# pairlab/SlotFormer

Hardware: AMD Instinct MI355X
Metric: rollout frames/sec at B=32, 128x128, 7 slots, 6+50 steps (SAVi-encode + SlotFormer rollout) (higher is better)
Workload: dtype f32 storage; matmul/conv on split-bf16 MFMA (bf16x3: hi*hi+hi*lo+lo*hi, f32 accumulate)

## Files before the change

include/slotformer_hip.h:

```cpp
#ifndef SLOTFORMER_HIP_H
#define SLOTFORMER_HIP_H
#include <stddef.h>

#ifdef __cplusplus
extern "C" {
#endif

int sf_version(void);
const char* sf_last_error_string(void);

int sf_get_precision(void);
int sf_set_precision(int mode);

int sf_profile_enable(int class_mask);
int sf_set_seam_fused(int on);
int sf_get_seam_fused(void);
int sf_set_ffn_rows64(int on);
int sf_get_ffn_rows64(void);
int sf_profile_sample(int every);
int sf_profile_read(int kernel_class, double* total_ms, long long* launches, double* work);


int sf_linear_f32(const float* A, int lda, const float* W, const float* bias, const float* ln_gamma,
                  const float* ln_beta, float ln_eps, const float* residual, int ldr, float* C, int ldc,
// ... 55 lines not shown
                        const float* std3, float* out, int F, int H0, int W0, int H, int W, int antialias, int max_blocks, void* stream);
int sf_resize_masks_nearest(const void* src, int src_is_u8, const void* tables, long long* out_i64, unsigned char* out_u8, int F, int H0,
                            int W0, int H, int W, void* stream);

enum { SF_EGRESS_TRUNC = 0, SF_EGRESS_NEAREST_EVEN = 1 };
enum { SF_EGRESS_F32_CHW = 0, SF_EGRESS_U8_CHW = 1, SF_EGRESS_U8_HWC = 2 };
enum { SF_EGRESS_IMG = 0, SF_EGRESS_SLOTS = 1, SF_EGRESS_IDS = 2 };
int sf_egress_frames_u8(const float* x, unsigned char* out, long long F, int H, int W, int hwc, int to_rgb, int rounding, void* stream);
typedef struct {
  int kind;
  int N;
  const void* a;
  const void* b;
  float scale;
  int ids_i64;
  int P;
  int history_len;
} sf_egress_tile;
int sf_egress_grid_shape(int K, int H, int W, int nrow, int padding, int border, int* CH, int* CW);
int sf_egress_grid(const sf_egress_tile* tiles, int n_entries, void* out, int out_mode, int T, int H, int W, int nrow, int padding,
                   float pad_value, int border, void* stream);
int sf_egress_draw_boxes(unsigned char* frames, const float* boxes, const unsigned char* pres, const unsigned char* palette, int P, int F, int M,
                         int H, int W, int width, void* stream);

int sf_pos_embed_table_f32(const float* grid, const float* dense_w, const float* dense_b, float* table, int HW,
                           int C, void* stream);

int sf_slot_attn_num_partials(int HW);
int sf_slot_attn_iter_f32(const float* k, const float* v, int ld, long long batch_stride, const float* q,
                          float* part_num, float* part_den, float* attn_out, int B, int HW, int N, int D,
                          float scale, float eps, void* stream);

int sf_slot_attn_iter_bf16(const void* k, const void* v, int ld, long long batch_stride, const float* q, float* part_num,
                           float* part_den, float* attn_out, int B, int HW, int N, int D, float scale, float eps, void* stream);

size_t sf_slot_attn_iter_bwd_workspace_bytes(int B, int HW, int N, int D);
int sf_slot_attn_iter_bwd_f32(const float* k, const float* v, int ld, long long batch_stride, const float* q,
                              const float* part_num, const float* part_den, int P, const float* d_updates, float* dk,
                              float* dv, int accumulate, float* dq, int B, int HW, int N, int D, float scale, float eps,
                              void* ws, size_t ws_bytes, void* stream);

int sf_slot_update_f32(const float* part_num, const float* part_den, int P, const float* slots_prev,
                       const float* gru_w_ih, const float* gru_w_hh, const float* gru_b_ih,
                       const float* gru_b_hh, const float* ln_g, const float* ln_b, const float* mlp_w1,
                       const float* mlp_b1, const float* mlp_w2, const float* mlp_b2, float* slots_out, int B,
                       int N, int D, int H, float ln_eps, void* stream);

int sf_slot_update_packed_f32(const float* part_num, const float* part_den, int P, const float* slots_prev,
                              const void* gru_ih_packed, const void* gru_hh_packed, const float* gru_b_ih,
                              const float* gru_b_hh, const float* ln_g, const float* ln_b, const void* mlp_w1_packed,
                              const float* mlp_b1, const void* mlp_w2_packed, const float* mlp_b2, float* slots_out,
                              const float* q_ln_g, const float* q_ln_b, const void* q_w_packed, float* q_out, int B, int N,
                              int D, int H, float ln_eps, void* stream);

int sf_mha_f32(const float* qkv, float* out, int B, int L, int Lq, int d_model, int num_heads, void* stream);

int sf_qkv_attention_f32(const float* x, const float* ln_gamma, const float* ln_beta, float ln_eps,
                         const float* in_proj_w, const float* in_proj_b, float* out, int B, int L, int Lq, int d_model,
                         int num_heads, void* stream);

int sf_lstm_pointwise_f32(const float* gates, const float* c_prev, float* h_out, float* c_out, int R, int H,
                          void* stream);

int sf_sample_dist_f32(const float* dist, const float* noise, float* out, int R, int D, void* stream);

int sf_bilinear_resize_f32(const float* in, float* out, long long R, int Hi, int Wi, int Ho, int Wo,
                           void* stream);

size_t sf_groupnorm1_workspace_bytes(int F);
int sf_groupnorm1_nhwc_f32(const float* x, const float* gamma, const float* beta, float* y, int F, int H, int W, int C,
                           float eps, int relu, int pixel_shuffle, void* ws, size_t ws_bytes, void* stream);
size_t sf_groupnorm1_bwd_workspace_bytes(int F, int H, int W, int C);
int sf_groupnorm1_nhwc_bwd_f32(const float* x, const float* gamma, const float* beta, const float* dy, float* dx, float* dgamma,
                               float* dbeta, int F, int H, int W, int C, float eps, int relu, int pixel_shuffle, void* ws,
                               size_t ws_bytes, void* stream);

int sf_slate_attention_f32(const float* q, const float* k, const float* v, float* out, int ldq, int ldk, int ldv, int ldo,
                           int B, int Lq, int Lk, int num_heads, int head_dim, int causal, void* stream);
size_t sf_slate_attention_bwd_workspace_bytes(int B, int Lq, int num_heads);
int sf_slate_attention_train_fwd_f32(const float* q, const float* k, const float* v, float* out, float* lse, int ldq, int ldk,
                                     int ldv, int ldo, long long q_bs, long long k_bs, long long v_bs, long long o_bs, int B,
                                     int Lq, int Lk, int num_heads, int head_dim, int causal, float dropout_p,
                                     unsigned long long seed, void* stream);
int sf_slate_attention_train_bwd_f32(const float* q, const float* k, const float* v, const float* out, const float* d_out,
                                     const float* lse, float* dq, float* dk, float* dv, int ldq, int ldk, int ldv, int ldo,
                                     long long q_bs, long long k_bs, long long v_bs, long long o_bs, int B, int Lq, int Lk,
                                     int num_heads, int head_dim, int causal, float dropout_p, unsigned long long seed, void* ws,
                                     size_t ws_bytes, void* stream);
int sf_slate_attention_bwd_f32(const float* q, const float* k, const float* v, const float* out, const float* d_out, float* dq,
                               float* dk, float* dv, int ldq, int ldk, int ldv, int ldo, long long q_bs, long long k_bs,
                               long long v_bs, long long o_bs, int B, int Lq, int Lk, int num_heads, int head_dim, int causal,
                               void* ws, size_t ws_bytes, void* stream);
int sf_slate_attention_strided_f32(const float* q, const float* k, const float* v, float* out, int ldq, int ldk, int ldv,
                                   int ldo, long long q_bs, long long k_bs, long long v_bs, long long o_bs, int B, int Lq,
                                   int Lk, int num_heads, int head_dim, int causal, void* stream);
int sf_embed_tokens_f32(const long long* idx, const float* tok_emb, const float* pos, float* out, int B, int L, int d,
                        void* stream);
int sf_argmax_rows_f32(const float* x, long long ld, long long* out, long long R, int V, void* stream);
int sf_cross_entropy_f32(const float* x, const long long* target, float* loss_rows, float* mean_out, long long R, int V,
                         void* stream);
int sf_softmax_rows_f32(const float* x, const float* add, float scale, float* y, long long R, int V, void* stream);
int sf_cross_entropy_bwd_f32(const float* x, const long long* target, const float* g, float* dx, long long R, int V, void* stream);
int sf_log_softmax_rows_f32(const float* x, float* y, long long R, int V, void* stream);
int sf_gumbel_softmax_rows_f32(const float* x, unsigned long long seed, float scale, float* y, long long R, int V, void* stream);
int sf_softmax_rows_bwd_f32(const float* y, const float* dy, float scale, float* dx, long long R, int V, void* stream);

// ... 322 lines not shown
```

slotformer_amd/_lib.py:

```python
import ctypes as C
import os

_HERE = os.path.dirname(os.path.abspath(__file__))
LIB_PATH = os.environ.get('SF_LIB_PATH') or os.path.join(_HERE, 'libslotformer_hip.so')

FP = C.c_void_p


class sf_tfm_layer(C.Structure):
    _fields_ = [(n, FP) for n in (
        'norm1_g', 'norm1_b', 'in_proj_w', 'in_proj_b', 'out_proj_w', 'out_proj_b',
        'norm2_g', 'norm2_b', 'lin1_w', 'lin1_b', 'lin2_w', 'lin2_b', 'lin1_packed', 'lin2_packed', 'attn_in_packed', 'attn_out_packed', 'tok_packed')]


class sf_rollouter(C.Structure):
    _fields_ = [(n, C.c_int) for n in (
        'num_slots', 'slot_size', 'd_model', 'num_layers', 'num_heads', 'ffn_dim', 'norm_first',
        'window_len', 'single_step')] + [(n, FP) for n in (
            'in_proj_w', 'in_proj_b', 'out_proj_w', 'out_proj_b', 'pe_tok')] + [
                ('layers', C.POINTER(sf_tfm_layer)), ('in_proj_packed', C.c_void_p), ('out_proj_packed', C.c_void_p)]


class sf_rollout_opts(C.Structure):
    _fields_ = [(n, C.c_int) for n in ('precision', 'seam_fused', 'ffn_rows', 'attn_heads_per_wg', 'attn_qkv_rows', 'ffn_tile', 'cus_available', 'layer_tok')]
# ... 100 lines not shown
    'sf_set_precision': (I, [I]),
    'sf_profile_enable': (I, [I]),
    'sf_profile_sample': (I, [I]),
    'sf_set_seam_fused': (I, [I]),
    'sf_get_seam_fused': (I, []),
    'sf_set_ffn_rows64': (I, [I]),
    'sf_get_ffn_rows64': (I, []),
    'sf_profile_read': (I, [I, C.POINTER(C.c_double), C.POINTER(C.c_longlong), C.POINTER(C.c_double)]),
    'sf_linear_f32': (I, [FP, I, FP, FP, FP, FP, F32, FP, I, FP, I, I, I, I, I, VP]),
    'sf_layernorm_f32': (I, [FP, FP, FP, FP, I, I, F32, VP]),
    'sf_conv2d_nchw_in_f32': (I, [FP, LL, FP, FP, FP, FP, I, I, I, I, I, I, I, I, VP]),
    'sf_conv2d_nhwc_f32': (I, [FP, FP, FP, FP, FP, I, I, I, I, I, I, I, VP]),
    'sf_pack_conv_weight_f32': (I, [FP, FP, I, I, I, VP]),
    'sf_pixel_feat_f32': (I, [FP] * 10 + [I, F32, I, VP]),
    'sf_conv_frag_bytes': (SZ, [I, I, I]),
    'sf_set_conv_fp16x2': (I, [I]),
    'sf_get_conv_fp16x2': (I, []),
    'sf_pack_conv_frag_weights': (I, [FP, VP, I, I, I, VP]),
    'sf_conv5x5_frag_f32': (I, [FP, VP, FP, FP, FP, I, I, I, I, VP]),
    'sf_conv5x5_ws_f32': (I, [FP, VP, FP, FP, FP, I, I, I, I, I, VP]),
    'sf_deconv_frag_bytes': (SZ, [I, I, I, I]),
    'sf_pack_deconv_frag_weights': (I, [FP, VP, I, I, I, I, VP]),
    'sf_deconv5x5s2_frag_f32': (I, [FP, VP, FP, FP, I, I, I, I, VP]),
    'sf_deconv5x5s2_head_frag_f32': (I, [FP, VP, FP, FP, FP, FP, I, I, I, VP]),
    'sf_decode_l0_expand_f32': (I, [FP, FP, FP, I, I, I, VP]),
    'sf_conv_transpose2d_nhwc_f32': (I, [FP, FP, FP, FP, I, I, I, I, I, I, I, I, VP]),
    'sf_pack_deconv_weight_f32': (I, [FP, FP, I, I, I, VP]),
    'sf_slot_broadcast_f32': (I, [FP, FP, FP, I, I, I, VP]),
    'sf_decode_combine_f32': (I, [FP, FP, FP, FP, I, I, I, VP]),
    'sf_savi_decode_workspace_bytes': (SZ, [C.POINTER(sf_savi_decoder), I]),
    'sf_savi_decode_f32': (I, [C.POINTER(sf_savi_decoder), FP, FP, FP, FP, I, VP, SZ, VP]),
    'sf_savi_decode_seg_f32': (I, [C.POINTER(sf_savi_decoder), FP, FP, FP, FP, VP, VP, F32, I, VP, SZ, VP]),
    'sf_decode_combine_seg_f32': (I, [FP, FP, FP, FP, VP, VP, F32, VP, I, I, I, VP]),
    'sf_postproc_mask_f32': (I, [FP, VP, VP, F32, VP, I, I, I, VP]),
    'sf_vp_metrics_workspace_bytes': (SZ, [I, I, I]),
    'sf_vp_image_metrics_f32': (I, [FP, FP, VP, VP, VP, I, I, I, I, VP, SZ, VP]),
    'sf_vp_mask_metrics': (I, [VP, VP, I, VP, FP, VP, VP, VP, VP, I, I, I, I, VP, SZ, VP]),
    'sf_vp_bbox_pr_f32': (I, [FP, VP, FP, VP, VP, I, I, I, F32, VP]),
    'sf_masks_to_boxes': (I, [VP, I, FP, VP, I, I, I, I, VP]),
    'sf_vp_mean_over_videos_f64': (I, [VP, VP, I, I, I, VP]),
    'sf_ingest_tables_bytes': (SZ, [I, I, I, I, I]),
    'sf_ingest_tables_host': (I, [VP, SZ, I, I, I, I, I]),
    'sf_ingest_frames_u8': (I, [VP, VP, I, VP, FP, FP, FP, I, I, I, I, I, I, I, VP]),
    'sf_resize_masks_nearest': (I, [VP, I, VP, VP, VP, I, I, I, I, I, VP]),
    'sf_egress_frames_u8': (I, [FP, VP, LL, I, I, I, I, I, VP]),
    'sf_egress_grid_shape': (I, [I, I, I, I, I, I, C.POINTER(I), C.POINTER(I)]),
    'sf_egress_grid': (I, [C.POINTER(sf_egress_tile), I, VP, I, I, I, I, I, I, F32, I, VP]),
    'sf_egress_draw_boxes': (I, [VP, FP, VP, VP, I, I, I, I, I, I, VP]),
    'sf_pos_embed_table_f32': (I, [FP, FP, FP, FP, I, I, VP]),
    'sf_slot_attn_num_partials': (I, [I]),
    'sf_slot_attn_iter_f32': (I, [FP, FP, I, LL, FP, FP, FP, FP, I, I, I, I, F32, F32, VP]),
    'sf_slot_update_f32': (I, [FP, FP, I, FP] + [FP] * 10 + [FP, I, I, I, I, F32, VP]),
    'sf_slot_update_packed_f32': (I, [FP, FP, I, FP, VP, VP, FP, FP, FP, FP, VP, FP, VP, FP, FP, FP, FP, VP, FP, I, I, I, I, F32, VP]),
    'sf_mha_f32': (I, [FP, FP, I, I, I, I, I, VP]),
    'sf_qkv_attention_f32': (I, [FP, FP, FP, F32, FP, FP, FP, I, I, I, I, I, VP]),
    'sf_lstm_pointwise_f32': (I, [FP, FP, FP, FP, I, I, VP]),
    'sf_sample_dist_f32': (I, [FP, FP, FP, I, I, VP]),
    'sf_bilinear_resize_f32': (I, [FP, FP, LL, I, I, I, I, VP]),
    'sf_rollout_workspace_bytes': (SZ, [C.POINTER(sf_rollouter), I]),
    'sf_rollout_f32': (I, [C.POINTER(sf_rollouter), FP, I, I, I, VP, SZ, VP]),
    'sf_rollout_opts_f32': (I, [C.POINTER(sf_rollouter), FP, I, I, I, VP, SZ, VP, C.POINTER(sf_rollout_opts)]),
    'sf_rollout_uses_seam': (I, [C.POINTER(sf_rollouter), I]),
    'sf_rollout_uses_seam_opts': (I, [C.POINTER(sf_rollouter), I, C.POINTER(sf_rollout_opts)]),
    'sf_rollout_is_fused': (I, [C.POINTER(sf_rollouter)]),
    'sf_rollout_tok_ok': (I, [C.POINTER(sf_rollouter)]),
    'sf_rollout_tok_layers': (I, [C.POINTER(sf_rollouter), I, C.POINTER(sf_rollout_opts)]),
    'sf_ffn_chunk_partials_f32': (I, [C.POINTER(sf_tfm_layer), FP, LL, FP, LL, I, I, I, VP]),
    'sf_attn_block_f32': (I, [C.POINTER(sf_tfm_layer), FP, FP, I, I, I, I, VP]),
    'sf_ffn_block_rows_f32': (I, [C.POINTER(sf_tfm_layer), FP, FP, I, I, VP]),
    'sf_set_layer_tok': (I, [I]),
    'sf_get_layer_tok': (I, []),
    'sf_layer_tok_packed_bytes': (SZ, []),
    'sf_layer_tok_packed_bytes_ex': (SZ, [I, I, I]),
    'sf_pack_layer_tok_weights': (I, [C.POINTER(sf_tfm_layer), VP, I, I, I, VP]),
    'sf_layer_tok_block_f32': (I, [C.POINTER(sf_tfm_layer), I, FP, FP, I, I, VP]),
    'sf_layer_tok_block_ex_f32': (I, [C.POINTER(sf_tfm_layer), I, I, I, I, FP, FP, I, I, VP]),
    'sf_debug_read_ts_layer_tok': (I, [C.POINTER(C.c_longlong)]),
    'sf_attn_rows_planes_bytes': (SZ, [I]),
    'sf_attn_block_rows_f32': (I, [C.POINTER(sf_tfm_layer), FP, FP, VP, I, I, I, VP]),
    'sf_slot_attn_iter_bwd_workspace_bytes': (SZ, [I, I, I, I]),
    'sf_slot_attn_iter_bwd_f32': (I, [FP, FP, I, LL, FP, FP, FP, I, FP, FP, FP, I, FP, I, I, I, I, F32, F32, VP, SZ, VP]),
    'sf_slot_attention_train_workspace_bytes': (SZ, [C.POINTER(sf_slot_attention), I, I, I]),
    'sf_slot_attention_train_fwd_f32': (I, [C.POINTER(sf_slot_attention), FP, FP, I, I, I, FP, VP, SZ, VP]),
    'sf_slot_attention_train_bwd_f32': (I, [C.POINTER(sf_slot_attention), FP, FP, FP, FP, C.POINTER(sf_slot_attention_grads), I, I, I,
                                            VP, SZ, VP]),
    'sf_savi_decode_train_workspace_bytes': (SZ, [C.POINTER(sf_savi_decoder), I]),
    'sf_savi_decode_train_fwd_f32': (I, [C.POINTER(sf_savi_decoder), FP, FP, FP, FP, I, VP, SZ, VP]),
    'sf_savi_decode_train_bwd_f32': (I, [C.POINTER(sf_savi_decoder), C.POINTER(C.c_void_p), FP, FP, FP, C.POINTER(sf_savi_decoder_grads),
                                         I, VP, SZ, VP]),
    'sf_savi_features_train_workspace_bytes': (SZ, [C.POINTER(sf_savi_features), I]),
    'sf_savi_features_train_fwd_f32': (I, [C.POINTER(sf_savi_features), FP, LL, I, FP, VP, SZ, VP]),
    'sf_savi_features_train_bwd_f32': (I, [C.POINTER(sf_savi_features), FP, LL, FP, C.POINTER(sf_savi_features_grads), I, VP, SZ, VP]),
    'sf_linear_bwd_workspace_bytes': (SZ, [LL, I, I]),
    'sf_linear_bwd_f32': (I, [FP, FP, FP, FP, FP, FP, FP, LL, I, I, I, VP, SZ, VP]),
    'sf_mha_train_fwd_f32': (I, [FP, FP, I, I, I, I, F32, C.c_ulonglong, VP]),
    'sf_mha_train_bwd_f32': (I, [FP, FP, FP, I, I, I, I, F32, C.c_ulonglong, VP]),
    'sf_dropout_f32': (I, [FP, FP, FP, LL, F32, C.c_ulonglong, VP]),
    'sf_adam_flat_f32': (I, [FP, FP, FP, FP, LL, I, F32, F32, F32, F32, VP]),
    'sf_grad_norm_workspace_bytes': (SZ, [LL]),
    'sf_grad_clip_coef_f32': (I, [FP, LL, F32, FP, VP, SZ, VP]),
    'sf_adam_flat_groups_f32': (I, [FP, FP, FP, FP, LL, I, C.POINTER(sf_adam_group), I, F32, F32, F32, FP, VP]),
    'sf_layernorm_bwd_workspace_bytes': (SZ, [I]),
    'sf_layernorm_bwd_f32': (I, [FP, FP, FP, FP, FP, FP, LL, I, F32, VP, SZ, VP]),
    'sf_rollout_train_workspace_bytes': (SZ, [C.POINTER(sf_rollouter), I, I]),
    'sf_rollout_train_fwd_f32': (I, [C.POINTER(sf_rollouter), FP, FP, I, I, F32, C.c_ulonglong, VP, SZ, VP]),
    'sf_rollout_train_bwd_f32': (I, [C.POINTER(sf_rollouter), FP, FP, C.POINTER(sf_rollouter_grads), I, I, F32,
# ... 177 lines not shown
```

slotformer_amd/csrc/slot_attn.hip:

```cpp
#include "sf_internal.h"
#include <stdlib.h>

#define SA_NMAX 8
#define SA_DMAX 256
#define SA_HMAX 512


template <int CTRL>
__device__ __forceinline__ float dpp_mov(float v) {
  return __int_as_float(__builtin_amdgcn_update_dpp(0, __float_as_int(v), CTRL, 0xf, 0xf, true));
}

__device__ __forceinline__ float wave_allsum(float v) {
  v += dpp_mov<0xB1>(v);
  v += dpp_mov<0x4E>(v);
  v += dpp_mov<0x141>(v);
  v += dpp_mov<0x140>(v);
  v += __shfl_xor(v, 16, 64);
  v += __shfl_xor(v, 32, 64);
  return v;
}

template <int VPT>
__global__ __launch_bounds__(256) void sa_attn_partial_kernel(
// ... 542 lines not shown
      const float v = su_sum(s_pa, ks, D2, j, r) + a.kd_b[j];
      s_hid[j * SU_R + r] = v;
      if (a.kdist_out && row < R) a.kdist_out[(long long)(row / N) * a.kdist_bs + (long long)(row % N) * D2 + j] = v;
    }
  }
  __syncthreads();
  for (int idx = t; idx < SU_R * D; idx += nt) {
    const int r = idx / D, d = idx - r * D, row = row0 + r;
    float v = s_hid[d * SU_R + r];
    if (a.noise && row < R)
      v += a.noise[(long long)(row / N) * a.noise_bs + (long long)(row % N) * D + d] * expf(s_hid[(D + d) * SU_R + r] * 0.5f);
    s_x[d * SU_R + r] = v;
    if (row < R) a.slots_out[(long long)row * D + d] = v;
  }
  __syncthreads();
  su_ln_stats(s_x, s_stat, D, ln_eps, wave, lane, nwaves);
  __syncthreads();
  for (int idx = t; idx < SU_R * D; idx += nt) {
    const int d = idx / SU_R, r = idx - d * SU_R;
    s_ln[idx] = (s_x[idx] - s_stat[2 * r]) * s_stat[2 * r + 1] * a.q_ln_g[d] + a.q_ln_b[d];
  }
  __syncthreads();
  su_gemm(a.q_w_t, D, D, s_ln, s_pa, t, nt);
  __syncthreads();
  {
    const int ks = su_kslices(nt, D, D);
    for (int idx = t; idx < SU_R * D; idx += nt) {
      const int r = idx / D, d = idx - r * D;
      if (row0 + r < R) a.q_out[(long long)(row0 + r) * D + d] = su_sum(s_pa, ks, D, d, r);
    }
  }
}

int sf_slot_prologue_ex(const float* prev, const float* init, const float* pm_ln_g, const float* pm_ln_b, const float* pm_w0_t,
                        const float* pm_b0, const float* pm_w2_t, const float* pm_b2, int norm_first, const float* kd_w_t,
                        const float* kd_b, const float* noise, long long noise_bs, float* kdist_out, long long kdist_bs,
                        const float* q_ln_g, const float* q_ln_b, const float* q_w_t, float* slots_out, float* q_out, int B,
                        int N, int D, float ln_eps, hipStream_t st) {
  if ((D % 64) != 0 || 2 * D > 768 || !kd_w_t || !kd_b || !q_w_t || !q_ln_g || !q_ln_b || !slots_out || !q_out || !init) return 1;
  if (prev && (!pm_ln_g || !pm_ln_b || !pm_w0_t || !pm_b0 || !pm_w2_t || !pm_b2)) return 1;
  if (B == 0) return 0;
  const int threads = 768, R = B * N, D2 = 2 * D;
  auto pmaxf = [&](int Nout, int K) { return su_kslices(threads, Nout, K) * Nout * SU_R; };
  int pmax = pmaxf(D2, D);
  if (pmaxf(D, D2) > pmax) pmax = pmaxf(D, D2);
  if (pmaxf(D, D) > pmax) pmax = pmaxf(D, D);
  const size_t lds = ((size_t)3 * D * SU_R + (size_t)D2 * SU_R + 2 * SU_R + (size_t)pmax) * sizeof(float);
  SF_TRY(sf_ensure_dyn_lds((const void*)sa_slot_prologue_kernel, lds));
  SpArgs a{prev, init, pm_ln_g, pm_ln_b, pm_w0_t, pm_b0, pm_w2_t, pm_b2, norm_first, kd_w_t, kd_b, noise, noise_bs, kdist_out,
           kdist_bs, q_ln_g, q_ln_b, q_w_t, slots_out, q_out};
  hipLaunchKernelGGL(sa_slot_prologue_kernel, dim3((R + SU_R - 1) / SU_R), dim3(threads), lds, st, a, R, N, D, pmax, ln_eps);
  SF_CHECK_LAUNCH();
  return 0;
}

int sf_sa_pick_partials(int HW) {
  if (HW % 256 == 0) return HW / 256;
  int P = HW / 128;
  while (P > 1 && (HW % P != 0 || (HW / P) % 16 != 0)) --P;
  if (P < 1) P = 1;
  return P;
}

extern "C" {

int sf_slot_attn_num_partials(int HW) { return sf_sa_pick_partials(HW); }

int sf_slot_attn_iter_f32(const float* k, const float* v, int ld, long long batch_stride, const float* q,
                          float* part_num, float* part_den, float* attn_out, int B, int HW, int N, int D,
                          float scale, float eps, void* stream) {
  return sf_slot_attn_iter_ex(k, v, ld, batch_stride, q, part_num, part_den, attn_out, (long long)N * HW, B, HW,
                              N, D, scale, eps, (hipStream_t)stream);
}
}

extern "C" int sf_slot_attn_iter_bf16(const void* k, const void* v, int ld, long long batch_stride, const float* q,
                                      float* part_num, float* part_den, float* attn_out, int B, int HW, int N, int D, float scale,
                                      float eps, void* stream) {
  SF_REQUIRE(k && v && q && part_num && part_den, "null pointer");
  SF_REQUIRE(B >= 0 && HW > 0 && (HW % 256) == 0 && N >= 1 && N <= SA_NMAX, "need 1 <= num_slots <= 8 and HW % 256 == 0");
  SF_REQUIRE(D == 64 || D == 128 || D == 192 || D == 256, "slot_size must be 64/128/192/256");
  SF_REQUIRE(ld >= D && (ld % 4) == 0 && (batch_stride % 4) == 0, "k/v rows must be 8-byte aligned");
  if (B == 0) return 0;
  const int P = sf_sa_pick_partials(HW);
  hipStream_t st = (hipStream_t)stream;
  dim3 grid(P, B), block(256);
  const __bf16* kb = (const __bf16*)k;
  const __bf16* vb = (const __bf16*)v;
  const long long abs_ = (long long)N * HW;
  sf_prof_begin(SF_K_SA_ITER, st, 2.0 * (double)B * HW * D * sizeof(__bf16));
#define SA_LAUNCHB(DD)                                                                                                   \
  hipLaunchKernelGGL((sa_attn_mfma_kernel<DD, __bf16>), grid, block, 0, st, kb, vb, ld, batch_stride, q, scale, eps, part_num, \
                     part_den, attn_out, abs_, HW, N, P)
  switch (D / 64) {
    case 1: SA_LAUNCHB(64); break;
    case 2: SA_LAUNCHB(128); break;
    case 3: SA_LAUNCHB(192); break;
    default: SA_LAUNCHB(256); break;
  }
#undef SA_LAUNCHB
  sf_prof_end(SF_K_SA_ITER, st);
  SF_CHECK_LAUNCH();
  return 0;
}

__device__ long long sa_ts[16];
// ... 225 lines not shown
```

slotformer_amd/csrc/slot_update_body.h:

```cpp
#pragma once
#include "sf_internal.h"


typedef float f32x16 __attribute__((ext_vector_type(16)));
typedef float f32x4 __attribute__((ext_vector_type(4)));
typedef __bf16 bf16x4 __attribute__((ext_vector_type(4)));
typedef __bf16 bf16x8 __attribute__((ext_vector_type(8)));

#ifdef UM_STAMPS
__device__ long long um_ts[16];
#define UMTS(i) do { if (block == 0 && threadIdx.x == 0) um_ts[i] = wall_clock64(); } while (0)
#else
#define UMTS(i) do { } while (0)
#endif

namespace {

constexpr int UM_D = 128, UM_H = 256, UM_ROWS = 32, UM_NT = 512;
constexpr int UM_DP = UM_D + 8, UM_HP = UM_H + 8;
constexpr int UM_FP = UM_D + 4;
constexpr int UV_BIH = 0, UV_BHH = 3 * UM_D, UV_LNG = 6 * UM_D, UV_LNB = 7 * UM_D, UV_B1 = 8 * UM_D, UV_B2 = 8 * UM_D + UM_H,
              UV_QG = 9 * UM_D + UM_H, UV_QB = 10 * UM_D + UM_H, UM_NV = 11 * UM_D + UM_H;
constexpr int UV_PG = UM_NV, UV_PBT = UV_PG + UM_D, UV_PB0 = UV_PBT + UM_D, UV_PB2 = UV_PB0 + UM_H, UV_KB = UV_PB2 + UM_D, UM_NV_NEXT = UV_KB + 2 * UM_D;
constexpr int UM_KP = 2 * UM_D + 8;
// ... 38 lines not shown
    acc = __builtin_amdgcn_mfma_f32_32x32x16_bf16(f.w[k][0], xl, acc, 0, 0, 0);
    acc = __builtin_amdgcn_mfma_f32_32x32x16_bf16(f.w[k][1], xh, acc, 0, 0, 0);
    acc = __builtin_amdgcn_mfma_f32_32x32x16_bf16(f.w[k][0], xh, acc, 0, 0, 0);
  }
}

struct UmArgs {
  const float *part_num, *part_den;
  int P;
  int pstep;
  const float* slots_prev;
  const uint4 *w_ih_p, *w_hh_p;
  const float *b_ih, *b_hh, *ln_g, *ln_b;
  const uint4* w1_p;
  const float* b1;
  const uint4* w2_p;
  const float* b2;
  float* slots_out;
  float* out2;
  long long out2_bs;
  const float *q_ln_g, *q_ln_b;
  const uint4* q_w_p;
  float* q_out;
  int R, N;
  float ln_eps;
  const float *pm_ln_g, *pm_ln_b;
  const uint4* pm_w0_p;
  const float* pm_b0;
  const uint4* pm_w2_p;
  const float* pm_b2;
  int pm_norm_first;
  const uint4* kd_w_p;
  const float* kd_b;
  const float* noise;
  long long noise_bs;
  float* kdist_out;
  long long kdist_bs;
  float* nx_slots;
};

}

constexpr size_t UM_LDS = (size_t)(4 * UM_ROWS * UM_DP + 2 * UM_ROWS * UM_HP) * 2
                          + (size_t)2 * UM_ROWS * UM_FP * 4
                          + (size_t)4 * 2 * 16 * 64 * 4
                          + (size_t)UM_ROWS * 64 * 4
                          + (size_t)UM_NV * 4;
constexpr size_t UM_LDS_NEXT = UM_LDS + (size_t)(UM_NV_NEXT - UM_NV) * 4;
static_assert((size_t)UM_ROWS * UM_KP * 4 <= (size_t)2 * UM_ROWS * UM_HP * 2, "kernel-distribution rows fit the hidden planes");

#define UM_G4(p) (*(f32x4 __attribute__((address_space(1)))*)(float __attribute__((address_space(1)))*)(p))
#define UM_CG4(p) (*(const f32x4 __attribute__((address_space(1)))*)(const float __attribute__((address_space(1)))*)(p))
#define UM_CGF(p) (*(const float __attribute__((address_space(1)))*)(p))
struct UmVar {
  const float *part_num, *part_den;
  int P, pstep;
  const float* slots_prev;
  float *slots_out, *out2, *q_out;
  const float* noise;
  float *kdist_out, *nx_slots;
  int R;
};

template <bool NEXT = false, class ArgsT = UmArgs, class VarT = UmVar>
__device__ __forceinline__ void um_rows(const ArgsT& a, const VarT& rv, float* um_lds_generic, const int block) {
  float* um_lds = (float*)(float __attribute__((address_space(3)))*)um_lds_generic;
  __bf16* Uh = (__bf16*)um_lds;
  __bf16* Ul = Uh + UM_ROWS * UM_DP;
  __bf16* Xh = Ul + UM_ROWS * UM_DP;
  __bf16* Xl = Xh + UM_ROWS * UM_DP;
  __bf16* Hh = Xl + UM_ROWS * UM_DP;
  __bf16* Hl = Hh + UM_ROWS * UM_HP;
  float* Fp = (float*)(Hl + UM_ROWS * UM_HP);
  float* Fn = Fp + UM_ROWS * UM_FP;
  float* EX = Fn + UM_ROWS * UM_FP;
  float* DN = EX + 4 * 2 * 16 * 64;
  float* PV = DN + UM_ROWS * 64;
  const int t = threadIdx.x, lane = t & 63, wave = t >> 6;
  const int row0 = block * UM_ROWS;
  const int cb = wave & 3, half = wave >> 2;
  const int tok = lane & 31, kg = lane >> 5;

  UMTS(0);
  float dnv[4];
#pragma unroll
  for (int i = 0; i < 4; ++i) {
    const int idx = t + UM_NT * i, r = idx >> 6, p = idx & 63, row = row0 + r;
    dnv[i] = 0.f;
    if (row < rv.R && p < rv.P) {
      const int b = row / a.N, n = row - b * a.N;
      dnv[i] = rv.part_den[((long long)b * rv.P * rv.pstep + (long long)p * rv.pstep) * a.N + n];
    }
  }
  const int ur = t >> 4, uc = (t & 15) * 8;
  const bool rok = row0 + ur < rv.R;
  const int urow = min(row0 + ur, rv.R - 1), ub = urow / a.N, un = urow - ub * a.N;
  const float* pn = rv.part_num + ((long long)ub * rv.P * rv.pstep * a.N + un) * UM_D + uc;
  const long long pst = (long long)rv.pstep * a.N * UM_D;
  f32x4 pa[8][2];
#pragma unroll
  for (int p = 0; p < 8; ++p) {
    const int pc = min(p, rv.P - 1);
    pa[p][0] = *(const f32x4*)(pn + pc * pst);
    pa[p][1] = *(const f32x4*)(pn + pc * pst + 4);
  }
  const f32x4 h0 = UM_CG4(rv.slots_prev + (long long)urow * UM_D + uc), h1 = UM_CG4(rv.slots_prev + (long long)urow * UM_D + uc + 4);
  constexpr int NPV = NEXT ? 5 : 4;
  float pvv[NPV];
#pragma unroll
  for (int i = 0; i < NPV; ++i) {
    const int j = t + UM_NT * i;
    float v = 0.f;
    if (j < UV_BHH) v = UM_CGF(a.b_ih + (j));
    else if (j < UV_LNG) v = UM_CGF(a.b_hh + (j - UV_BHH));
    else if (j < UV_LNB) v = UM_CGF(a.ln_g + (j - UV_LNG));
    else if (j < UV_B1) v = UM_CGF(a.ln_b + (j - UV_LNB));
    else if (j < UV_B2) v = UM_CGF(a.b1 + (j - UV_B1));
    else if (j < UV_QG) v = UM_CGF(a.b2 + (j - UV_B2));
    else if (j < UV_QB) v = rv.q_out ? UM_CGF(a.q_ln_g + (j - UV_QG)) : 0.f;
    else if (j < UM_NV) v = rv.q_out ? UM_CGF(a.q_ln_b + (j - UV_QB)) : 0.f;
    else if constexpr (NEXT) {
      if (j < UV_PBT) v = UM_CGF(a.pm_ln_g + (j - UV_PG));
      else if (j < UV_PB0) v = UM_CGF(a.pm_ln_b + (j - UV_PBT));
      else if (j < UV_PB2) v = UM_CGF(a.pm_b0 + (j - UV_PB0));
      else if (j < UV_KB) v = UM_CGF(a.pm_b2 + (j - UV_PB2));
      else v = UM_CGF(a.kd_b + (j - UV_KB));
    }
    pvv[i] = v;
  }
  UmFrags<8> fa, fb;
  um_load(fa, a.w_ih_p, 12, half * 4 + cb, 0, lane);
#pragma unroll
  for (int i = 0; i < 4; ++i) {
    DN[t + UM_NT * i] = dnv[i];
    if (t + UM_NT * i < (NEXT ? UM_NV_NEXT : UM_NV)) PV[t + UM_NT * i] = pvv[i];
  }
  if constexpr (NEXT) PV[t + UM_NT * 4] = pvv[4];
  f32x4 n0 = {0.f, 0.f, 0.f, 0.f}, n1 = n0;
#pragma unroll
  for (int p = 0; p < 8; ++p)
    if (p < rv.P) {
      n0 += pa[p][0];
      n1 += pa[p][1];
    }
  if (rv.P > 8) {
#pragma unroll
    for (int p = 0; p < 8; ++p) {
      const int pc = min(8 + p, rv.P - 1);
      pa[p][0] = *(const f32x4*)(pn + pc * pst);
      pa[p][1] = *(const f32x4*)(pn + pc * pst + 4);
    }
  }
  um_load(fb, a.w_hh_p, 12, half * 4 + cb, 0, lane);
  if (rv.P > 8) {
#pragma unroll
    for (int p = 0; p < 8; ++p)
      if (8 + p < rv.P) {
        n0 += pa[p][0];
        n1 += pa[p][1];
      }
    for (int p = 16; p < rv.P; ++p) {
      n0 += *(const f32x4*)(pn + p * pst);
      n1 += *(const f32x4*)(pn + p * pst + 4);
    }
  }
  UMTS(1);
  __syncthreads();
  UMTS(2);
  {
    float den = 0.f;
    for (int p = 0; p < rv.P; ++p) den += DN[ur * 64 + p];
    const f32x4 zero4 = {0.f, 0.f, 0.f, 0.f};
    um_split4(Uh, Ul, ur * UM_DP + uc, rok ? n0 / den : zero4);
    um_split4(Uh, Ul, ur * UM_DP + uc + 4, rok ? n1 / den : zero4);
    um_split4(Xh, Xl, ur * UM_DP + uc, rok ? h0 : zero4);
    um_split4(Xh, Xl, ur * UM_DP + uc + 4, rok ? h1 : zero4);
    *(f32x4*)(Fp + ur * UM_FP + uc) = rok ? h0 : zero4;
    *(f32x4*)(Fp + ur * UM_FP + uc + 4) = rok ? h1 : zero4;
  }
  __syncthreads();

  UMTS(3);
  f32x16 g1, g2;
#pragma unroll
  for (int r = 0; r < 16; ++r) g1[r] = g2[r] = 0.f;
  um_gemm(g1, fa, Uh, Ul, UM_DP, 0, lane);
  um_load(fa, half == 0 ? a.w_ih_p : a.w_hh_p, 12, 8 + cb, 0, lane);
  um_gemm(g1, fb, Xh, Xl, UM_DP, 0, lane);
  UmFrags<8> fm;
  um_load(fm, a.w1_p, 8, wave, 0, lane);
  um_gemm(g2, fa, half == 0 ? Uh : Xh, half == 0 ? Ul : Xl, UM_DP, 0, lane);
  UMTS(4);
  if (half == 1) {
#pragma unroll
    for (int g = 0; g < 4; ++g) {
      const int c = 32 * cb + 8 * g + 4 * kg;
      const f32x4 bz = *(const f32x4*)(PV + UV_BIH + UM_D + c) + *(const f32x4*)(PV + UV_BHH + UM_D + c), bn = *(const f32x4*)(PV + UV_BHH + 2 * UM_D + c);
#pragma unroll
      for (int q = 0; q < 4; ++q) {
        EX[((cb * 2 + 0) * 16 + 4 * g + q) * 64 + lane] = um_sigmoid(g1[4 * g + q] + bz[q]);
        EX[((cb * 2 + 1) * 16 + 4 * g + q) * 64 + lane] = g2[4 * g + q] + bn[q];
      }
    }
  }
  else {
#pragma unroll
    for (int g = 0; g < 4; ++g) {
      const int c = 32 * cb + 8 * g + 4 * kg;
      const f32x4 br = *(const f32x4*)(PV + UV_BIH + c) + *(const f32x4*)(PV + UV_BHH + c);
#pragma unroll
      for (int q = 0; q < 4; ++q) g1[4 * g + q] = um_sigmoid(g1[4 * g + q] + br[q]);
    }
  }
  __syncthreads();
  if (half == 0) {
#pragma unroll
    for (int g = 0; g < 4; ++g) {
      const int c = 32 * cb + 8 * g + 4 * kg;
      const f32x4 bn = *(const f32x4*)(PV + UV_BIH + 2 * UM_D + c);
      const f32x4 hp = *(const f32x4*)(Fp + tok * UM_FP + c);
      f32x4 hn;
#pragma unroll
      for (int q = 0; q < 4; ++q) {
        const float rr = g1[4 * g + q];
        const float z = EX[((cb * 2 + 0) * 16 + 4 * g + q) * 64 + lane], ghn = EX[((cb * 2 + 1) * 16 + 4 * g + q) * 64 + lane];
        const float nn = um_tanh(g2[4 * g + q] + bn[q] + rr * ghn);
        hn[q] = (1.f - z) * nn + z * hp[q];
      }
      *(f32x4*)(Fn + tok * UM_FP + c) = hn;
    }
  }
  __syncthreads();

  UMTS(5);
  UmFrags<8> f2;
  um_load(f2, a.w2_p, 4, cb, half * 8, lane);
  UmFrags<8> fp0, fp2, fk;
  {
    const f32x4 v0 = *(const f32x4*)(Fn + ur * UM_FP + uc), v1 = *(const f32x4*)(Fn + ur * UM_FP + uc + 4);
    const float mu = sf_sum16(((v0[0] + v0[1]) + (v0[2] + v0[3])) + ((v1[0] + v1[1]) + (v1[2] + v1[3]))) / (float)UM_D;
    const f32x4 d0 = v0 - mu, d1 = v1 - mu;
    const float var = sf_sum16(((d0[0] * d0[0] + d0[1] * d0[1]) + (d0[2] * d0[2] + d0[3] * d0[3])) +
                               ((d1[0] * d1[0] + d1[1] * d1[1]) + (d1[2] * d1[2] + d1[3] * d1[3]))) / (float)UM_D;
    const float rs = 1.0f / sqrtf(var + a.ln_eps);
    um_split4(Xh, Xl, ur * UM_DP + uc, d0 * rs * *(const f32x4*)(PV + UV_LNG + uc) + *(const f32x4*)(PV + UV_LNB + uc));
    um_split4(Xh, Xl, ur * UM_DP + uc + 4, d1 * rs * *(const f32x4*)(PV + UV_LNG + uc + 4) + *(const f32x4*)(PV + UV_LNB + uc + 4));
  }
  __syncthreads();

  UMTS(6);
#pragma unroll
  for (int r = 0; r < 16; ++r) g1[r] = 0.f;
  um_gemm(g1, fm, Xh, Xl, UM_DP, 0, lane);
#pragma unroll
  for (int g = 0; g < 4; ++g) {
    const int c = 32 * wave + 8 * g + 4 * kg;
    const f32x4 bb = *(const f32x4*)(PV + UV_B1 + c);
    const f32x4 hv = {fmaxf(g1[4 * g] + bb[0], 0.f), fmaxf(g1[4 * g + 1] + bb[1], 0.f), fmaxf(g1[4 * g + 2] + bb[2], 0.f),
                      fmaxf(g1[4 * g + 3] + bb[3], 0.f)};
    um_split4(Hh, Hl, tok * UM_HP + c, hv);
  }
  __syncthreads();

  UMTS(7);
  UmFrags<4> fq;
  if (rv.q_out) um_load(fq, a.q_w_p, 4, cb, half * 4, lane);
  if constexpr (NEXT) um_load(fp0, a.pm_w0_p, 8, wave, 0, lane);
#pragma unroll
  for (int r = 0; r < 16; ++r) g2[r] = 0.f;
  um_gemm(g2, f2, Hh, Hl, UM_HP, half * 8, lane);
  if constexpr (NEXT) um_load(fp2, a.pm_w2_p, 4, cb, half * 8, lane);
  if (half == 1) {
#pragma unroll
    for (int r = 0; r < 16; ++r) EX[(cb * 2 * 16 + r) * 64 + lane] = g2[r];
  }
  __syncthreads();
  if (half == 0) {
    const int row = row0 + tok;
    const int b = min(row, rv.R - 1) / a.N, n = min(row, rv.R - 1) - b * a.N;
#pragma unroll
    for (int g = 0; g < 4; ++g) {
      const int c = 32 * cb + 8 * g + 4 * kg;
      const f32x4 bb = *(const f32x4*)(PV + UV_B2 + c), hn = *(const f32x4*)(Fn + tok * UM_FP + c);
// ... 145 lines not shown
```

slotformer_amd/csrc/slot_update_mfma.hip:

```cpp
#include "slot_update_body.h"

template <bool NEXT>
__global__ __launch_bounds__(UM_NT) void sa_slot_update_mfma_kernel(UmArgs a) {
  extern __shared__ __attribute__((aligned(16))) float um_lds[];
  um_body<NEXT>(a, um_lds, blockIdx.x);
}

bool sf_slot_update_mfma_ok(int D, int H, int P) { return D == UM_D && H == UM_H && P >= 1 && P <= 64; }

int sf_slot_update_mfma_ex(const float* part_num, const float* part_den, int P, const float* slots_prev, const void* gru_ih_p,
                           const void* gru_hh_p, const float* gru_b_ih, const float* gru_b_hh, const float* ln_g, const float* ln_b,
                           const void* w1_p, const float* b1, const void* w2_p, const float* b2, float* slots_out, float* out2,
                           long long out2_bs, const float* q_ln_g, const float* q_ln_b, const void* q_w_p, float* q_out, int B, int N,
                           float ln_eps, hipStream_t st, const SfNextStep* next, int p_step) {
  SF_REQUIRE(part_num && part_den && slots_prev && slots_out && gru_ih_p && gru_hh_p && gru_b_ih && gru_b_hh && ln_g && ln_b && w1_p &&
                 b1 && w2_p && b2, "sf_slot_update_mfma_ex: null pointer");
  SF_REQUIRE(!next || (q_out && next->pm_ln_g && next->pm_ln_b && next->pm_w0_p && next->pm_b0 && next->pm_w2_p && next->pm_b2 && next->kd_w_p &&
                       next->kd_b && next->slots && next->slots != slots_out),
             "sf_slot_update_mfma_ex: the next-step form needs q_out, the predictor / kernel-distribution operands and its own slot buffer");
  SF_REQUIRE(q_out == nullptr || (q_ln_g && q_ln_b && q_w_p), "q projection requested without its weights");
  SF_REQUIRE(N >= 1 && P >= 1 && P <= 64 && (p_step == 1 || (p_step == 2 && P % 2 == 0)), "bad slot shape");
  if (B == 0) return 0;
  static_assert(UM_LDS_NEXT <= 160 * 1024, "slot update: LDS budget");
  SF_TRY(next ? sf_ensure_dyn_lds((const void*)sa_slot_update_mfma_kernel<true>, (size_t)(UM_LDS_NEXT))
              : sf_ensure_dyn_lds((const void*)sa_slot_update_mfma_kernel<false>, (size_t)(UM_LDS)));
  UmArgs a;
  memset(&a, 0, sizeof(a));
  a.part_num = part_num; a.part_den = part_den; a.P = P / p_step; a.pstep = p_step; a.slots_prev = slots_prev;
  a.w_ih_p = (const uint4*)gru_ih_p; a.w_hh_p = (const uint4*)gru_hh_p; a.b_ih = gru_b_ih; a.b_hh = gru_b_hh; a.ln_g = ln_g; a.ln_b = ln_b;
  a.w1_p = (const uint4*)w1_p; a.b1 = b1; a.w2_p = (const uint4*)w2_p; a.b2 = b2; a.slots_out = slots_out; a.out2 = out2; a.out2_bs = out2_bs;
  a.q_ln_g = q_ln_g; a.q_ln_b = q_ln_b; a.q_w_p = (const uint4*)q_w_p; a.q_out = q_out; a.R = B * N; a.N = N; a.ln_eps = ln_eps;
  const int R = B * N;
  if (next) {
    a.pm_ln_g = next->pm_ln_g; a.pm_ln_b = next->pm_ln_b; a.pm_w0_p = (const uint4*)next->pm_w0_p; a.pm_b0 = next->pm_b0;
    a.pm_w2_p = (const uint4*)next->pm_w2_p; a.pm_b2 = next->pm_b2; a.pm_norm_first = next->norm_first; a.kd_w_p = (const uint4*)next->kd_w_p;
    a.kd_b = next->kd_b; a.noise = next->noise; a.noise_bs = next->noise_bs; a.kdist_out = next->kdist_out; a.kdist_bs = next->kdist_bs;
    a.nx_slots = next->slots;
  }
  sf_prof_begin(SF_K_SA_UPDATE, st,
                2.0 * R * ((double)6 * UM_D * UM_D + 2.0 * UM_D * UM_H + (q_out ? (double)UM_D * UM_D : 0.0) + (next ? 6.0 * UM_D * UM_D : 0.0)));
  if (next)
    hipLaunchKernelGGL(sa_slot_update_mfma_kernel<true>, dim3((R + UM_ROWS - 1) / UM_ROWS), dim3(UM_NT), UM_LDS_NEXT, st, a);
  else
    hipLaunchKernelGGL(sa_slot_update_mfma_kernel<false>, dim3((R + UM_ROWS - 1) / UM_ROWS), dim3(UM_NT), UM_LDS, st, a);
  sf_prof_end(SF_K_SA_UPDATE, st);
  SF_CHECK_LAUNCH();
  return 0;
}

extern "C" int sf_slot_update_packed_f32(const float* part_num, const float* part_den, int P, const float* slots_prev, const void* gru_ih_packed,
                                         const void* gru_hh_packed, const float* gru_b_ih, const float* gru_b_hh, const float* ln_g,
                                         const float* ln_b, const void* mlp_w1_packed, const float* mlp_b1, const void* mlp_w2_packed,
                                         const float* mlp_b2, float* slots_out, const float* q_ln_g, const float* q_ln_b,
                                         const void* q_w_packed, float* q_out, int B, int N, int D, int H, float ln_eps, void* stream) {
  if (sf_slot_update_wide_ok(D, H, P))
    return sf_slot_update_wide_ex(part_num, part_den, P, slots_prev, gru_ih_packed, gru_hh_packed, gru_b_ih, gru_b_hh, ln_g, ln_b, mlp_w1_packed,
                                  mlp_b1, mlp_w2_packed, mlp_b2, slots_out, nullptr, 0, q_ln_g, q_ln_b, q_w_packed, q_out, B, N, ln_eps,
                                  (hipStream_t)stream);
  SF_REQUIRE(sf_slot_update_mfma_ok(D, H, P),
             "sf_slot_update_packed_f32: slot size 128 with slot MLP size 256, or 192 with 384, and at most 64 partial records");
  return sf_slot_update_mfma_ex(part_num, part_den, P, slots_prev, gru_ih_packed, gru_hh_packed, gru_b_ih, gru_b_hh, ln_g, ln_b, mlp_w1_packed,
                                mlp_b1, mlp_w2_packed, mlp_b2, slots_out, nullptr, 0, q_ln_g, q_ln_b, q_w_packed, q_out, B, N, ln_eps,
                                (hipStream_t)stream);
}

#ifdef UM_STAMPS
extern "C" int sf_debug_read_ts_um(long long* out16) {
  hipError_t e = hipMemcpyFromSymbol(out16, HIP_SYMBOL(um_ts), sizeof(long long) * 16);
  return e == hipSuccess ? 0 : (int)e;
}
#endif
```

Measured before the change: 650,900.

## Rebalance GRU gate epilogue across both halves and make slot-update loads wave-uniform

The GRU epilogue in the slot-update kernel now has both wave halves exchange half their gate results through LDS, so each half finishes half of the new-state columns. Previously one half did all of the tanh and blend work while the other sat idle after a barrier. The partial-record count and wave index become wave-uniform scalars, which allows unpredicated full-unrolled partial sums when there are at least 8 or 16 records. Parameter-vector staging now picks one source pointer per wave instead of running a long per-thread branch chain. New C entry points expose the extended slot update and the slot prologue, which adds API surface but no new hot-path behaviour.

After: 657,000 (median of 5 runs). No clear change (+0.9%).

```diff
diff --git a/include/slotformer_hip.h b/include/slotformer_hip.h
--- a/include/slotformer_hip.h
+++ b/include/slotformer_hip.h
@@ -131,6 +131,20 @@
                               const float* mlp_b1, const void* mlp_w2_packed, const float* mlp_b2, float* slots_out,
                               const float* q_ln_g, const float* q_ln_b, const void* q_w_packed, float* q_out, int B, int N,
                               int D, int H, float ln_eps, void* stream);
+int sf_slot_update_packed_ex_f32(const float* part_num, const float* part_den, int P, int p_step, const float* slots_prev,
+                                 const void* gru_ih_packed, const void* gru_hh_packed, const float* gru_b_ih, const float* gru_b_hh,
+                                 const float* ln_g, const float* ln_b, const void* mlp_w1_packed, const float* mlp_b1,
+                                 const void* mlp_w2_packed, const float* mlp_b2, float* slots_out, float* out2, long long out2_bs,
+                                 const float* q_ln_g, const float* q_ln_b, const void* q_w_packed, float* q_out, const float* pm_ln_g,
+                                 const float* pm_ln_b, const void* pm_w0_packed, const float* pm_b0, const void* pm_w2_packed,
+                                 const float* pm_b2, int norm_first, const void* kd_w_packed, const float* kd_b, const float* noise,
+                                 long long noise_bs, float* kdist_out, long long kdist_bs, float* next_slots, int B, int N, int D, int H,
+                                 float ln_eps, void* stream);
+int sf_slot_prologue_f32(const float* prev, const float* init, const float* pm_ln_g, const float* pm_ln_b, const float* pm_w0_t,
+                         const float* pm_b0, const float* pm_w2_t, const float* pm_b2, int norm_first, const float* kd_w_t,
+                         const float* kd_b, const float* noise, long long noise_bs, float* kdist_out, long long kdist_bs,
+                         const float* q_ln_g, const float* q_ln_b, const float* q_w_t, float* slots_out, float* q_out, int B, int N, int D,
+                         float ln_eps, void* stream);
 
 int sf_mha_f32(const float* qkv, float* out, int B, int L, int Lq, int d_model, int num_heads, void* stream);
 
diff --git a/slotformer_amd/_lib.py b/slotformer_amd/_lib.py
--- a/slotformer_amd/_lib.py
+++ b/slotformer_amd/_lib.py
@@ -176,6 +176,9 @@
     'sf_slot_attn_iter_f32': (I, [FP, FP, I, LL, FP, FP, FP, FP, I, I, I, I, F32, F32, VP]),
     'sf_slot_update_f32': (I, [FP, FP, I, FP] + [FP] * 10 + [FP, I, I, I, I, F32, VP]),
     'sf_slot_update_packed_f32': (I, [FP, FP, I, FP, VP, VP, FP, FP, FP, FP, VP, FP, VP, FP, FP, FP, FP, VP, FP, I, I, I, I, F32, VP]),
+    'sf_slot_update_packed_ex_f32': (I, [FP, FP, I, I, FP, VP, VP, FP, FP, FP, FP, VP, FP, VP, FP, FP, FP, LL, FP, FP, VP, FP, FP, FP, VP, FP, VP, FP, I,
+                                         VP, FP, FP, LL, FP, LL, FP, I, I, I, I, F32, VP]),
+    'sf_slot_prologue_f32': (I, [FP] * 8 + [I, FP, FP, FP, LL, FP, LL, FP, FP, FP, FP, FP, I, I, I, F32, VP]),
     'sf_mha_f32': (I, [FP, FP, I, I, I, I, I, VP]),
     'sf_qkv_attention_f32': (I, [FP, FP, FP, F32, FP, FP, FP, I, I, I, I, I, VP]),
     'sf_lstm_pointwise_f32': (I, [FP, FP, FP, FP, I, I, VP]),
diff --git a/slotformer_amd/csrc/slot_attn.hip b/slotformer_amd/csrc/slot_attn.hip
--- a/slotformer_amd/csrc/slot_attn.hip
+++ b/slotformer_amd/csrc/slot_attn.hip
@@ -618,6 +618,18 @@
   hipLaunchKernelGGL(sa_slot_prologue_kernel, dim3((R + SU_R - 1) / SU_R), dim3(threads), lds, st, a, R, N, D, pmax, ln_eps);
   SF_CHECK_LAUNCH();
   return 0;
+}
+
+extern "C" int sf_slot_prologue_f32(const float* prev, const float* init, const float* pm_ln_g, const float* pm_ln_b, const float* pm_w0_t,
+                                    const float* pm_b0, const float* pm_w2_t, const float* pm_b2, int norm_first, const float* kd_w_t, const float* kd_b,
+                                    const float* noise, long long noise_bs, float* kdist_out, long long kdist_bs, const float* q_ln_g,
+                                    const float* q_ln_b, const float* q_w_t, float* slots_out, float* q_out, int B, int N, int D, float ln_eps,
+                                    void* stream) {
+  const int rc = sf_slot_prologue_ex(prev, init, pm_ln_g, pm_ln_b, pm_w0_t, pm_b0, pm_w2_t, pm_b2, norm_first, kd_w_t, kd_b, noise, noise_bs, kdist_out,
+                                     kdist_bs, q_ln_g, q_ln_b, q_w_t, slots_out, q_out, B, N, D, ln_eps, (hipStream_t)stream);
+  SF_REQUIRE(rc != 1, "sf_slot_prologue_f32: needs a slot size that is a multiple of 64 up to 384, init, the kernel-distribution and q operands, and the "
+                      "predictor's operands with prev");
+  return rc;
 }
 
 int sf_sa_pick_partials(int HW) {
diff --git a/slotformer_amd/csrc/slot_update_body.h b/slotformer_amd/csrc/slot_update_body.h
--- a/slotformer_amd/csrc/slot_update_body.h
+++ b/slotformer_amd/csrc/slot_update_body.h
@@ -114,6 +114,29 @@
 #define UM_G4(p) (*(f32x4 __attribute__((address_space(1)))*)(float __attribute__((address_space(1)))*)(p))
 #define UM_CG4(p) (*(const f32x4 __attribute__((address_space(1)))*)(const float __attribute__((address_space(1)))*)(p))
 #define UM_CGF(p) (*(const float __attribute__((address_space(1)))*)(p))
+template <bool NEXT, class ArgsT>
+__device__ __forceinline__ const float* um_pv_src(const ArgsT& a, bool has_q, int seg) {
+  static_assert(UV_BHH % 128 == 0 && UV_LNG % 128 == 0 && UV_B1 % 128 == 0 && UV_B2 % 128 == 0 && UV_QG % 128 == 0 && UM_NV % 128 == 0 &&
+                    UV_PB0 % 128 == 0 && UV_PB2 % 128 == 0 && UV_KB % 128 == 0 && UM_NT == 512, "parameter-vector staging: one vector per wave and round");
+  const int j = seg * 128;
+  if (j < UV_BHH) return a.b_ih - UV_BIH;
+  if (j < UV_LNG) return a.b_hh - UV_BHH;
+  if (j < UV_LNB) return a.ln_g - UV_LNG;
+  if (j < UV_B1) return a.ln_b - UV_LNB;
+  if (j < UV_B2) return a.b1 - UV_B1;
+  if (j < UV_QG) return a.b2 - UV_B2;
+  if (j < UV_QB) return has_q ? a.q_ln_g - UV_QG : nullptr;
+  if (j < UM_NV) return has_q ? a.q_ln_b - UV_QB : nullptr;
+  if constexpr (NEXT) {
+    if (j < UV_PBT) return a.pm_ln_g - UV_PG;
+    if (j < UV_PB0) return a.pm_ln_b - UV_PBT;
+    if (j < UV_PB2) return a.pm_b0 - UV_PB0;
+    if (j < UV_KB) return a.pm_b2 - UV_PB2;
+    if (j < UM_NV_NEXT) return a.kd_b - UV_KB;
+  }
+  return nullptr;
+}
+
 struct UmVar {
   const float *part_num, *part_den;
   int P, pstep;
@@ -145,11 +168,13 @@
 
   UMTS(0);
   float dnv[4];
+  const int wv = __builtin_amdgcn_readfirstlane(wave);
+  const int nrec = __builtin_amdgcn_readfirstlane(rv.P);
 #pragma unroll
   for (int i = 0; i < 4; ++i) {
-    const int idx = t + UM_NT * i, r = idx >> 6, p = idx & 63, row = row0 + r;
+    const int r = wv + 8 * i, p = lane, row = row0 + r;
     dnv[i] = 0.f;
-    if (row < rv.R && p < rv.P) {
+    if (row < rv.R && p < nrec) {
       const int b = row / a.N, n = row - b * a.N;
       dnv[i] = rv.part_den[((long long)b * rv.P * rv.pstep + (long long)p * rv.pstep) * a.N + n];
     }
@@ -162,7 +187,7 @@
   f32x4 pa[8][2];
 #pragma unroll
   for (int p = 0; p < 8; ++p) {
-    const int pc = min(p, rv.P - 1);
+    const int pc = min(p, nrec - 1);
     pa[p][0] = *(const f32x4*)(pn + pc * pst);
     pa[p][1] = *(const f32x4*)(pn + pc * pst + 4);
   }
@@ -171,24 +196,11 @@
   float pvv[NPV];
 #pragma unroll
   for (int i = 0; i < NPV; ++i) {
-    const int j = t + UM_NT * i;
-    float v = 0.f;
-    if (j < UV_BHH) v = UM_CGF(a.b_ih + (j));
-    else if (j < UV_LNG) v = UM_CGF(a.b_hh + (j - UV_BHH));
-    else if (j < UV_LNB) v = UM_CGF(a.ln_g + (j - UV_LNG));
-    else if (j < UV_B1) v = UM_CGF(a.ln_b + (j - UV_LNB));
-    else if (j < UV_B2) v = UM_CGF(a.b1 + (j - UV_B1));
-    else if (j < UV_QG) v = UM_CGF(a.b2 + (j - UV_B2));
-    else if (j < UV_QB) v = rv.q_out ? UM_CGF(a.q_ln_g + (j - UV_QG)) : 0.f;
-    else if (j < UM_NV) v = rv.q_out ? UM_CGF(a.q_ln_b + (j - UV_QB)) : 0.f;
-    else if constexpr (NEXT) {
-      if (j < UV_PBT) v = UM_CGF(a.pm_ln_g + (j - UV_PG));
-      else if (j < UV_PB0) v = UM_CGF(a.pm_ln_b + (j - UV_PBT));
-      else if (j < UV_PB2) v = UM_CGF(a.pm_b0 + (j - UV_PB0));
-      else if (j < UV_KB) v = UM_CGF(a.pm_b2 + (j - UV_PB2));
-      else v = UM_CGF(a.kd_b + (j - UV_KB));
-    }
-    pvv[i] = v;
+    const int wp = wv >> 1;
+    const float* src = nullptr;
+#pragma unroll
+    for (int k = 0; k < 4; ++k) src = wp == k ? um_pv_src<NEXT>(a, rv.q_out != nullptr, 4 * i + k) : src;
+    pvv[i] = src ? UM_CGF(src + (t + UM_NT * i)) : 0.f;
   }
   UmFrags<8> fa, fb;
   um_load(fa, a.w_ih_p, 12, half * 4 + cb, 0, lane);
@@ -199,29 +211,45 @@
   }
   if constexpr (NEXT) PV[t + UM_NT * 4] = pvv[4];
   f32x4 n0 = {0.f, 0.f, 0.f, 0.f}, n1 = n0;
-#pragma unroll
-  for (int p = 0; p < 8; ++p)
-    if (p < rv.P) {
+  if (nrec >= 8) {
+#pragma unroll
+    for (int p = 0; p < 8; ++p) {
       n0 += pa[p][0];
       n1 += pa[p][1];
     }
-  if (rv.P > 8) {
+  } else {
+#pragma unroll
+    for (int p = 0; p < 8; ++p)
+      if (p < nrec) {
+        n0 += pa[p][0];
+        n1 += pa[p][1];
+      }
+  }
+  if (nrec > 8) {
 #pragma unroll
     for (int p = 0; p < 8; ++p) {
-      const int pc = min(8 + p, rv.P - 1);
+      const int pc = min(8 + p, nrec - 1);
       pa[p][0] = *(const f32x4*)(pn + pc * pst);
       pa[p][1] = *(const f32x4*)(pn + pc * pst + 4);
     }
   }
   um_load(fb, a.w_hh_p, 12, half * 4 + cb, 0, lane);
-  if (rv.P > 8) {
+  if (nrec >= 16) {
+#pragma unroll
+    for (int p = 0; p < 8; ++p) {
+      n0 += pa[p][0];
+      n1 += pa[p][1];
+    }
+  } else if (nrec > 8) {
 #pragma unroll
     for (int p = 0; p < 8; ++p)
-      if (8 + p < rv.P) {
+      if (8 + p < nrec) {
         n0 += pa[p][0];
         n1 += pa[p][1];
       }
-    for (int p = 16; p < rv.P; ++p) {
+  }
+  if (nrec > 16) {
+    for (int p = 16; p < nrec; ++p) {
       n0 += *(const f32x4*)(pn + p * pst);
       n1 += *(const f32x4*)(pn + p * pst + 4);
     }
@@ -231,7 +259,7 @@
   UMTS(2);
   {
     float den = 0.f;
-    for (int p = 0; p < rv.P; ++p) den += DN[ur * 64 + p];
+    for (int p = 0; p < nrec; ++p) den += DN[ur * 64 + p];
     const f32x4 zero4 = {0.f, 0.f, 0.f, 0.f};
     um_split4(Uh, Ul, ur * UM_DP + uc, rok ? n0 / den : zero4);
     um_split4(Uh, Ul, ur * UM_DP + uc + 4, rok ? n1 / den : zero4);
@@ -260,8 +288,12 @@
       const f32x4 bz = *(const f32x4*)(PV + UV_BIH + UM_D + c) + *(const f32x4*)(PV + UV_BHH + UM_D + c), bn = *(const f32x4*)(PV + UV_BHH + 2 * UM_D + c);
 #pragma unroll
       for (int q = 0; q < 4; ++q) {
-        EX[((cb * 2 + 0) * 16 + 4 * g + q) * 64 + lane] = um_sigmoid(g1[4 * g + q] + bz[q]);
-        EX[((cb * 2 + 1) * 16 + 4 * g + q) * 64 + lane] = g2[4 * g + q] + bn[q];
+        g1[4 * g + q] = um_sigmoid(g1[4 * g + q] + bz[q]);
+        g2[4 * g + q] = g2[4 * g + q] + bn[q];
+        if (g < 2) {
+          EX[((cb * 2 + 0) * 16 + 4 * g + q) * 64 + lane] = g1[4 * g + q];
+          EX[((cb * 2 + 0) * 16 + 8 + 4 * g + q) * 64 + lane] = g2[4 * g + q];
+        }
       }
     }
   }
@@ -269,28 +301,33 @@
 #pragma unroll
     for (int g = 0; g < 4; ++g) {
       const int c = 32 * cb + 8 * g + 4 * kg;
-      const f32x4 br = *(const f32x4*)(PV + UV_BIH + c) + *(const f32x4*)(PV + UV_BHH + c);
-#pragma unroll
-      for (int q = 0; q < 4; ++q) g1[4 * g + q] = um_sigmoid(g1[4 * g + q] + br[q]);
-    }
-  }
-  __syncthreads();
-  if (half == 0) {
-#pragma unroll
-    for (int g = 0; g < 4; ++g) {
-      const int c = 32 * cb + 8 * g + 4 * kg;
-      const f32x4 bn = *(const f32x4*)(PV + UV_BIH + 2 * UM_D + c);
-      const f32x4 hp = *(const f32x4*)(Fp + tok * UM_FP + c);
-      f32x4 hn;
+      const f32x4 br = *(const f32x4*)(PV + UV_BIH + c) + *(const f32x4*)(PV + UV_BHH + c), bn = *(const f32x4*)(PV + UV_BIH + 2 * UM_D + c);
 #pragma unroll
       for (int q = 0; q < 4; ++q) {
-        const float rr = g1[4 * g + q];
-        const float z = EX[((cb * 2 + 0) * 16 + 4 * g + q) * 64 + lane], ghn = EX[((cb * 2 + 1) * 16 + 4 * g + q) * 64 + lane];
-        const float nn = um_tanh(g2[4 * g + q] + bn[q] + rr * ghn);
-        hn[q] = (1.f - z) * nn + z * hp[q];
-      }
-      *(f32x4*)(Fn + tok * UM_FP + c) = hn;
-    }
+        g1[4 * g + q] = um_sigmoid(g1[4 * g + q] + br[q]);
+        g2[4 * g + q] = g2[4 * g + q] + bn[q];
+        if (g >= 2) {
+          EX[((cb * 2 + 1) * 16 + 4 * (g - 2) + q) * 64 + lane] = g1[4 * g + q];
+          EX[((cb * 2 + 1) * 16 + 8 + 4 * (g - 2) + q) * 64 + lane] = g2[4 * g + q];
+        }
+      }
+    }
+  }
+  __syncthreads();
+#pragma unroll
+  for (int gg = 0; gg < 2; ++gg) {
+    const int c = 32 * cb + 8 * (2 * half + gg) + 4 * kg;
+    const f32x4 hp = *(const f32x4*)(Fp + tok * UM_FP + c);
+    f32x4 hn;
+#pragma unroll
+    for (int q = 0; q < 4; ++q) {
+      const float ea = EX[((cb * 2 + half) * 16 + 4 * gg + q) * 64 + lane], eb = EX[((cb * 2 + half) * 16 + 8 + 4 * gg + q) * 64 + lane];
+      const float rr = half == 0 ? g1[4 * gg + q] : ea, gin = half == 0 ? g2[4 * gg + q] : eb;
+      const float z = half == 0 ? ea : g1[8 + 4 * gg + q], ghn = half == 0 ? eb : g2[8 + 4 * gg + q];
+      const float nn = um_tanh(gin + rr * ghn);
+      hn[q] = (1.f - z) * nn + z * hp[q];
+    }
+    *(f32x4*)(Fn + tok * UM_FP + c) = hn;
   }
   __syncthreads();
 
diff --git a/slotformer_amd/csrc/slot_update_mfma.hip b/slotformer_amd/csrc/slot_update_mfma.hip
--- a/slotformer_amd/csrc/slot_update_mfma.hip
+++ b/slotformer_amd/csrc/slot_update_mfma.hip
@@ -64,6 +64,25 @@
                                 (hipStream_t)stream);
 }
 
+extern "C" int sf_slot_update_packed_ex_f32(const float* part_num, const float* part_den, int P, int p_step, const float* slots_prev,
+                                            const void* gru_ih_packed, const void* gru_hh_packed, const float* gru_b_ih, const float* gru_b_hh,
+                                            const float* ln_g, const float* ln_b, const void* mlp_w1_packed, const float* mlp_b1,
+                                            const void* mlp_w2_packed, const float* mlp_b2, float* slots_out, float* out2, long long out2_bs,
+                                            const float* q_ln_g, const float* q_ln_b, const void* q_w_packed, float* q_out, const float* pm_ln_g,
+                                            const float* pm_ln_b, const void* pm_w0_packed, const float* pm_b0, const void* pm_w2_packed,
+                                            const float* pm_b2, int norm_first, const void* kd_w_packed, const float* kd_b, const float* noise,
+                                            long long noise_bs, float* kdist_out, long long kdist_bs, float* next_slots, int B, int N, int D, int H,
+                                            float ln_eps, void* stream) {
+  SF_REQUIRE(sf_slot_update_mfma_ok(D, H, P), "sf_slot_update_packed_ex_f32: slot size 128 with slot MLP size 256, and at most 64 partial records");
+  SfNextStep nx;
+  nx.pm_ln_g = pm_ln_g; nx.pm_ln_b = pm_ln_b; nx.pm_w0_p = pm_w0_packed; nx.pm_b0 = pm_b0; nx.pm_w2_p = pm_w2_packed; nx.pm_b2 = pm_b2;
+  nx.norm_first = norm_first; nx.kd_w_p = kd_w_packed; nx.kd_b = kd_b; nx.noise = noise; nx.noise_bs = noise_bs; nx.kdist_out = kdist_out;
+  nx.kdist_bs = kdist_bs; nx.slots = next_slots;
+  return sf_slot_update_mfma_ex(part_num, part_den, P, slots_prev, gru_ih_packed, gru_hh_packed, gru_b_ih, gru_b_hh, ln_g, ln_b, mlp_w1_packed,
+                                mlp_b1, mlp_w2_packed, mlp_b2, slots_out, out2, out2_bs, q_ln_g, q_ln_b, q_w_packed, q_out, B, N, ln_eps,
+                                (hipStream_t)stream, pm_w0_packed ? &nx : nullptr, p_step);
+}
+
 #ifdef UM_STAMPS
 extern "C" int sf_debug_read_ts_um(long long* out16) {
   hipError_t e = hipMemcpyFromSymbol(out16, HIP_SYMBOL(um_ts), sizeof(long long) * 16);
```
